# jfjlaros/HUMID

Measured on AMD Instinct MI355X. Metric: reads/sec deduplicated, 10M PE150 UMI=8 d=1, higher is better.
Workload: dtype u64; 1 GPU; 10000000 reads/GPU x 1 GPU (one shuffled read set of 10000000 reads, sliced by input order), PE150 UMI=8 in header -> 24-nt packed words (8+8+8), d=1, directional clustering; synthetic molecules=N/4, family 1+Geom(3), p_sub=1e-3, p_N=1e-4; reads_per_gpu=10000000, word_nt=24, distance=1, method=directional

## Files before the change

humid_amd/csrc/humid_hip.hip:

```cpp
#include "pipeline.hip.h"
#include "kernels_best.hip.h"
#include "kernels_consensus.hip.h"

static std::string g_err;
extern "C" __attribute__((visibility("hidden"))) void humid_set_global_error(const char *text) { g_err = text ? text : ""; }

extern "C" {

uint32_t humid_abi_version(void) { return HUMID_ABI_VERSION; }

int humid_device_count(void) {
  int n = 0;
  if (hipGetDeviceCount(&n) != hipSuccess) return 0;
  return n;
}

const char *humid_last_error(const humid_ctx *ctx) { return ctx ? ctx->err.c_str() : g_err.c_str(); }

int humid_ctx_create(humid_ctx **out, int device, void *stream) {
  humid_ctx *c = nullptr;
  if (!out) return fail(nullptr, HUMID_E_INVALID, "out is null");
  *out = nullptr;
  int ndev = 0;
  hipError_t e = hipGetDeviceCount(&ndev);
// ... 112 lines not shown
    c->kr_force_log2 = (u32)value;
    return HUMID_OK;
  }
  if (strcmp(key, "whitelist_coop") == 0) {
    c->wl_coop = value != 0;
    return HUMID_OK;
  }
  if (strcmp(key, "tile_partition") == 0) {
    c->use_tile_partition = value != 0;
    return HUMID_OK;
  }
  if (strcmp(key, "coop_big") == 0) {
    c->coop_big = value != 0;
    return HUMID_OK;
  }
  if (strcmp(key, "kernel_timing") == 0) {
    c->kev_on = value != 0;
    return HUMID_OK;
  }
  if (strcmp(key, "test_fail_before_gather") == 0) {
    c->x_test_fail_after = (int)value;
    return HUMID_OK;
  }
  if (strcmp(key, "records8") == 0) {
    c->use_rec8 = value != 0;
    return HUMID_OK;
  }
  if (strcmp(key, "compact_graph") == 0) {
    c->use_compact = value != 0;
    return HUMID_OK;
  }
  if (strcmp(key, "group_buckets") == 0) {
    c->group_buckets = value != 0;
    return HUMID_OK;
  }
  if (strcmp(key, "padded_partition") == 0) {
    c->pt_padded = value != 0;
    return HUMID_OK;
  }
  if (strcmp(key, "force_comm") == 0) {
    c->force_comm = value != 0;
    return HUMID_OK;
  }
  if (strcmp(key, "bucket_walk") == 0) {
    if (value < 0 || value > (1 << 24)) return fail(c, HUMID_E_INVALID, "bucket_walk must be 0 (no limit) .. 2^24");
    c->walk_max = (u32)value;
    return HUMID_OK;
  }
  if (strcmp(key, "plan_segments") == 0) {
    if (value < 0 || value > 32) return fail(c, HUMID_E_INVALID, "plan_segments must be 0 (auto) .. 32");
    c->force_segments = (u32)value;
    return HUMID_OK;
  }
  return fail(c, HUMID_E_INVALID, "unknown option '%s'", key);
}

int humid_dedup_run_device(humid_ctx *c, const uint64_t *d_words, const uint8_t *d_filtered,
                           uint64_t n_reads, uint32_t word_nt, uint32_t distance, uint32_t method,
                           uint32_t *d_cluster_id, uint8_t *d_keep, humid_summary *summary) {
  if (!c) return fail(nullptr, HUMID_E_INVALID, "ctx is null");
  return with_word_type(word_nt, [&](auto *w) {
    return run_device(c, (decltype(w))d_words, d_filtered, n_reads, word_nt, distance, method, d_cluster_id, d_keep, summary);
  });
}

int humid_dedup_run_grouped_device(humid_ctx *c, const uint64_t *d_words, const uint32_t *d_group,
// ... 806 lines not shown
```

humid_amd/csrc/kernels_cgraph.hip.h:

```cpp
#ifndef HUMID_KERNELS_CGRAPH_HIP_H
#define HUMID_KERNELS_CGRAPH_HIP_H

#include "common.hip.h"
#include "kernels_graph.hip.h"
#include "kernels_cluster.hip.h"

#define ER_REGIONS 64u
#define ER_STRIDE 32u
struct EdgeRegs {
  u64 *e;
  u32 cap_r;
  u32 *cur;
  const u64 *far;
  u32 n_far;
};
__device__ __forceinline__ u32 er_count(const EdgeRegs &er, u32 r) {
  if (r == ER_REGIONS) return er.n_far;
  const u32 c = er.cur[r * ER_STRIDE];
  return c < er.cap_r ? c : er.cap_r;
}
__device__ __forceinline__ u64 *er_at(const EdgeRegs &er, u32 r, u32 k) {
  return r == ER_REGIONS ? (u64 *)er.far + k : er.e + (size_t)r * er.cap_r + k;
}

// ... 27 lines not shown
    return (u32)(__popc(x.x) + __popc(x.y) + __popc(x.z) + __popc(x.w) + __popc(y.x) + __popc(y.y) + __popc(y.z) + __popc(y.w));
  }
};

static __global__ void __launch_bounds__(256)
k_bits_blocks(const u32 *__restrict__ bits, u32 n_blk, u32 *__restrict__ cnt) {
  HUMID_GUARD_LAST_VGPR();
  const u32 b = blockIdx.x * blockDim.x + threadIdx.x;
  if (b > n_blk) return;
  if (b == n_blk) { cnt[b] = 0; return; }
  const uint4 *p = (const uint4 *)(bits + 8 * (size_t)b);
  const uint4 x = p[0], y = p[1];
  cnt[b] = (u32)(__popc(x.x) + __popc(x.y) + __popc(x.z) + __popc(x.w) + __popc(y.x) + __popc(y.y) + __popc(y.z) + __popc(y.w));
}

#define ZERO_MAX 8
struct ZeroList {
  u32 *p[ZERO_MAX];
  u32 n[ZERO_MAX];
};
static __global__ void __launch_bounds__(256)
k_zero_many(ZeroList z) {
  HUMID_GUARD_LAST_VGPR();
  const u32 stride = gridDim.x * blockDim.x;
#pragma unroll
  for (u32 q = 0; q < ZERO_MAX; q++) {
    u32 *p = z.p[q];
    const u32 n = z.n[q];
    for (u32 i = blockIdx.x * blockDim.x + threadIdx.x; i < n; i += stride) p[i] = 0;
  }
}

#define PA_PPT 4u
template <bool PASS0, class WT>
__global__ void __launch_bounds__(256)
k_pairs_append(const WT *__restrict__ W, const u32 *__restrict__ V, u32 n, WT mask, EarlierMasksT<WT> em, u32 cb,
               u32 distance, u32 walk_max, EdgeRegs er, u32 *bits, ull *big, u32 *overflow,
               const u32 *__restrict__ n_valid = nullptr) {
  HUMID_GUARD_LAST_VGPR();
  __shared__ u32 lds[8];
  __shared__ u32 s_base;
  PH_DECL;
  PH(0);
  if (n_valid && *n_valid < n) n = *n_valid;
  const u32 i0 = blockIdx.x * (PA_PPT * 256u) + threadIdx.x;
  u32 found[PA_PPT], first_off[PA_PPT], jend[PA_PPT];
  WT wi[PA_PPT], w1[PA_PPT];
#pragma unroll
  for (u32 q = 0; q < PA_PPT; q++) {
    const u32 i = i0 + q * 256u;
    found[q] = 0; first_off[q] = 0; jend[q] = 0;
    if (i < n) {
      wi[q] = W[i];
      w1[q] = W[i + 1 < n ? i + 1 : i];
    }
  }
  u32 total_found = 0;
#pragma unroll
  for (u32 q = 0; q < PA_PPT; q++) {
    const u32 i = i0 + q * 256u;
    if (i >= n) continue;
    jend[q] = (walk_max && n - i > walk_max + 1) ? i + walk_max + 1 : n;
    u32 j = i + 1;
    for (; j < jend[q]; j++) {
      const WT x = w_xor(wi[q], j == i + 1 ? w1[q] : W[j]);
      if (w_hits(x, mask)) break;
      if (w_mismatch(x) > distance) continue;
      bool first = true;
#pragma unroll
      for (u32 t = 0; t < MAX_COMBOS; t++)
        first = first && !(t < cb && !w_hits(x, em.m[t]));
      if (!first) continue;
      if (!found[q]) first_off[q] = j - i;
      found[q]++;
    }
    if (big && j == jend[q] && jend[q] < n && !w_hits(w_xor(wi[q], W[jend[q]]), mask)) atomicOr(big, 1ull << cb);
    total_found += found[q];
  }
  PH(1);
  const u32 lane = threadIdx.x & 63, wv = threadIdx.x >> 6;
  u32 incl = total_found;
  incl = wave_incl_scan(incl);
  if (lane == 63) lds[wv] = incl;
  __syncthreads();
  u32 before = 0, total = 0;
#pragma unroll
  for (u32 k = 0; k < 4; k++) { if (k < wv) before += lds[k]; total += lds[k]; }
  PH(2);
  if (total == 0) { PH(3); PH(4); PH_END(5, 4, (blockIdx.x & 15u) == 5u); return; }
  const u32 region = blockIdx.x % ER_REGIONS;
  if (threadIdx.x == 0) s_base = atomicAdd(&er.cur[region * ER_STRIDE], total);
  __syncthreads();
  PH(3);
  if (threadIdx.x == 0) { PH(4); PH_END(5, 4, (blockIdx.x & 15u) == 5u); }
  if (!total_found) return;
  u32 at = s_base + before + incl - total_found;
  if (at + total_found > er.cap_r) { *overflow = 1; if (at >= er.cap_r) return; }
  u64 *out = er.e + (size_t)region * er.cap_r;
#pragma unroll
  for (u32 q = 0; q < PA_PPT; q++) {
    if (!found[q]) continue;
    const u32 i = i0 + q * 256u;
    const u32 ri = PASS0 ? i : V[i];
    auto emit = [&](u32 j) {
      if (at >= er.cap_r) return;
      const u32 rj = PASS0 ? j : V[j];
      out[at++] = ri < rj ? (((u64)ri << 32) | rj) : (((u64)rj << 32) | ri);
      atomicOr(&bits[rj >> 5], 1u << (rj & 31));
    };
    atomicOr(&bits[ri >> 5], 1u << (ri & 31));
    if (found[q] == 1) { emit(i + first_off[q]); continue; }
    for (u32 j = i + first_off[q]; j < jend[q]; j++) {
      const WT x = w_xor(wi[q], W[j]);
      if (w_hits(x, mask)) break;
      if (w_mismatch(x) > distance) continue;
      bool first = true;
#pragma unroll
      for (u32 t = 0; t < MAX_COMBOS; t++)
        first = first && !(t < cb && !w_hits(x, em.m[t]));
      if (first) emit(j);
    }
  }
}

static __global__ void __launch_bounds__(256)
k_mark_pairs(const u64 *__restrict__ pairs, u32 n_pairs, u32 n_leaves, u32 *bits, u32 *bad) {
  HUMID_GUARD_LAST_VGPR();
  const u32 k = blockIdx.x * blockDim.x + threadIdx.x;
  if (k >= n_pairs) return;
  const u64 e = pairs[k];
  const u32 a = (u32)(e >> 32), b = (u32)e;
  if (a >= n_leaves || b >= n_leaves || a == b) { *bad = 1; return; }
  atomicOr(&bits[a >> 5], 1u << (a & 31));
  atomicOr(&bits[b >> 5], 1u << (b & 31));
}

static __global__ void __launch_bounds__(256)
k_nodes_init(BitRank br, u32 n_words, const u32 *__restrict__ s_cnt, u32 *__restrict__ nodes, u32 *__restrict__ ncnt,
             u32 *__restrict__ deg, u32 *__restrict__ parent, u32 *__restrict__ csize, u32 *__restrict__ cur, u32 n_blk) {
  HUMID_GUARD_LAST_VGPR();
  const u32 w = blockIdx.x * blockDim.x + threadIdx.x;
  if (w == 0) deg[br.blk[n_blk]] = 0;
  if (w >= n_words) return;
  u32 x = br.bits[w];
  if (!x) return;
  u32 c = br_rank(br, w << 5);
  while (x) {
    const u32 bit = (u32)__ffs((int)x) - 1u;
    x &= x - 1u;
    const u32 u = (w << 5) | bit;
    nodes[c] = u;
    if (s_cnt) ncnt[c] = s_cnt[u];
    deg[c] = 0; parent[c] = c; csize[c] = 0; cur[c] = 0;
    c++;
  }
}
// ... 236 lines not shown
```

humid_amd/csrc/kernels_part.hip.h:

```cpp
#ifndef HUMID_KERNELS_PART_HIP_H
#define HUMID_KERNELS_PART_HIP_H

#include "common.hip.h"
#include "kernels_count.hip.h"

#define PT_THREADS 1024u
#define PT_TILE 8192u
#define PT_IPT (PT_TILE / PT_THREADS)
#define PT_MAXBINS 512u
#define PT_MAXBINS1 1024u

struct PtInput {
  const u64 *words;
  const u8 *filtered;
  u64 rlo, rhi;
  u32 check_range;
  PartKeyOp key;
};
__device__ __forceinline__ bool pt_load(const PtInput &in, u32 r, u64 &key) {
  if (in.filtered && in.filtered[r]) return false;
  const u64 w = in.words[r];
  if (in.check_range && (w < in.rlo || w > in.rhi)) return false;
  key = in.key(w);
  return true;
// ... 196 lines not shown
    const u32 bin = sbin[s];
    const u32 within = s - loff[bin];
    if (within >= room[bin]) continue;
    const u32 d = goff[bin] + within;
    k_out[d] = skey[s];
    v_out[d] = sval[s];
  }
}

template <class SRC>
__global__ void __launch_bounds__(1024)
k_pt_hist2(SRC src, const u64 *__restrict__ k_in, const u32 *__restrict__ tprefix, const u32 *__restrict__ cbase, u32 d1,
           u32 d2, u32 *__restrict__ hist_fine, u32 cap1) {
  HUMID_GUARD_LAST_VGPR();
  __shared__ u32 h[PT_MAXBINS];
  __shared__ u32 s_c, s_beg, s_cnt;
  if (blockIdx.x >= tprefix[1u << d1]) return;
  const u32 nb = 1u << d2;
  if (threadIdx.x == 0) {
    u32 c, b, n;
    pt_tile_of(tprefix, cbase, 1u << d1, blockIdx.x, cap1, c, b, n);
    s_c = c; s_beg = b; s_cnt = n;
  }
  for (u32 b = threadIdx.x; b < nb; b += PT_THREADS) h[b] = 0;
  __syncthreads();
  const u32 beg = s_beg, n = s_cnt;
  for (u32 j = threadIdx.x; j < n; j += PT_THREADS)
    atomicAdd(&h[(u32)(src.key(k_in[beg + j]) >> (64 - d1 - d2)) & (nb - 1)], 1u);
  __syncthreads();
  for (u32 b = threadIdx.x; b < nb; b += PT_THREADS)
    if (h[b]) atomicAdd(&hist_fine[(s_c << d2) | b], h[b]);
}

#define GF_THREADS 1024u
#define GF_MAXBITS 15u
#define GF_SMALL 7872u
#define GF_MID 32768u
template <class SRC, int SIZE>
__global__ void __launch_bounds__(GF_THREADS, SIZE == 0 ? 8 : 4)
k_group_fine(SRC src, const u64 *__restrict__ k_in, const u32 *__restrict__ v_in, const u32 *__restrict__ cbase, u32 d1,
             u32 d2, u64 *__restrict__ k_out, u32 *__restrict__ v_out, u32 cap1) {
  HUMID_GUARD_LAST_VGPR();
  constexpr bool BIG = SIZE == 2;
  constexpr u32 INV_WORDS = SIZE == 0 ? GF_SMALL / 2u + 16u : (1u << (GF_MAXBITS - 1)) + 16u;
  __shared__ u32 gf_lds[BIG ? (1u << GF_MAXBITS) + 16 : (1u << (GF_MAXBITS - 1)) + INV_WORDS];
  const u32 nb = 1u << d2, c = blockIdx.x;
  PH_DECL;
  PH(0);
  const u32 beg = cbase[c], end = cbase[c + 1];
  if (beg >= end) return;
  const u32 n = end - beg;
  if ((n <= GF_SMALL ? 0 : (n <= GF_MID ? 1 : 2)) != SIZE) return;
  const u32 ibeg = cap1 ? c * cap1 : beg;
  k_in += ibeg; v_in += ibeg; k_out += beg; v_out += beg;
  u32 *wsum = BIG ? gf_lds + (1u << GF_MAXBITS) : gf_lds + (1u << (GF_MAXBITS - 1)) + INV_WORDS - 16;
  const u32 lane = threadIdx.x & 63, wv = threadIdx.x >> 6;
  auto fine = [&](u64 w) { return (u32)(src.key(w) >> (64 - d1 - d2)) & (nb - 1); };
  if (!BIG) {
    unsigned short *inv = (unsigned short *)(gf_lds + (1u << (GF_MAXBITS - 1)));
    constexpr u32 GF_RPT = 8;
    u64 kk[GF_RPT];
    u32 ff[GF_RPT];
    if constexpr (SIZE == 0) {
#pragma unroll
      for (u32 q = 0; q < GF_RPT; q++) {
        const u32 j = threadIdx.x + q * GF_THREADS;
        kk[q] = j < n ? k_in[j] : 0ull;
      }
    }
    for (u32 b = threadIdx.x; b < (1u << (GF_MAXBITS - 1)); b += GF_THREADS) gf_lds[b] = 0;
    __syncthreads();
    PH(1);
    if constexpr (SIZE == 0) {
#pragma unroll
      for (u32 q = 0; q < GF_RPT; q++) {
        const u32 j = threadIdx.x + q * GF_THREADS;
        ff[q] = fine(kk[q]);
        if (j < n) atomicAdd(&gf_lds[ff[q] >> 1], 1u << (16 * (ff[q] & 1)));
// ... 31 lines not shown
    PH(4);
    if constexpr (SIZE == 0) {
      u32 oldq[GF_RPT];
#pragma unroll
      for (u32 q = 0; q < GF_RPT; q++) {
        const u32 j = threadIdx.x + q * GF_THREADS;
        oldq[q] = j < n ? atomicAdd(&gf_lds[ff[q] >> 1], 1u << (16 * (ff[q] & 1))) : 0u;
      }
#pragma unroll
      for (u32 q = 0; q < GF_RPT; q++) {
        const u32 j = threadIdx.x + q * GF_THREADS;
        if (j < n) inv[(oldq[q] >> (16 * (ff[q] & 1))) & 0xffffu] = (unsigned short)j;
      }
      PH(5);
      __syncthreads();
      PH(6);
      u32 jj[GF_RPT], vo[GF_RPT];
      u64 ko[GF_RPT];
#pragma unroll
      for (u32 t = 0; t < GF_RPT; t++) {
        const u32 q = threadIdx.x + t * GF_THREADS;
        jj[t] = q < n ? inv[q] : 0u;
      }
#pragma unroll
      for (u32 t = 0; t < GF_RPT; t++) {
        const u32 q = threadIdx.x + t * GF_THREADS;
        if (q < n) { ko[t] = k_in[jj[t]]; vo[t] = v_in[jj[t]]; }
      }
#pragma unroll
      for (u32 t = 0; t < GF_RPT; t++) {
        const u32 q = threadIdx.x + t * GF_THREADS;
        if (q < n) { k_out[q] = ko[t]; v_out[q] = vo[t]; }
      }
      PH(7);
      PH_END(4, 7, (c & 7u) == 3u);
      return;
    }
    for (u32 j = threadIdx.x; j < n; j += GF_THREADS) {
      const u32 f = fine(k_in[j]);
      const u32 old = atomicAdd(&gf_lds[f >> 1], 1u << (16 * (f & 1)));
      inv[(old >> (16 * (f & 1))) & 0xffffu] = (unsigned short)j;
    }
    __syncthreads();
    for (u32 q = threadIdx.x; q < n; q += GF_THREADS) {
      const u32 j = inv[q];
      k_out[q] = k_in[j];
      v_out[q] = v_in[j];
    }
    return;
  }
  for (u32 b = threadIdx.x; b < nb; b += GF_THREADS) gf_lds[b] = 0;
  __syncthreads();
  for (u32 j = threadIdx.x; j < n; j += GF_THREADS) atomicAdd(&gf_lds[fine(k_in[j])], 1u);
  __syncthreads();
  const u32 per = nb >= GF_THREADS ? nb / GF_THREADS : 1u;
  const u32 b0 = threadIdx.x * per;
  u32 mine = 0;
  if (b0 < nb)
    for (u32 q = 0; q < per; q++) mine += gf_lds[b0 + q];
  u32 incl = mine;
  incl = wave_incl_scan(incl);
  if (lane == 63) wsum[wv] = incl;
  __syncthreads();
  u32 run = incl - mine;
  for (u32 q = 0; q < wv; q++) run += wsum[q];
  if (b0 < nb)
// ... 141 lines not shown
```

humid_amd/csrc/pipeline.hip.h:

```cpp
#ifndef HUMID_PIPELINE_HIP_H
#define HUMID_PIPELINE_HIP_H

#include <fcntl.h>
#include <sys/mman.h>
#include <sys/stat.h>
#include <unistd.h>

#include <atomic>
#include <cerrno>
#include <chrono>
#include <type_traits>
#include <utility>

#include "common.hip.h"
#include "prims.hip.h"
#include "kernels_count.hip.h"
#include "kernels_part.hip.h"
#include "kernels_part8.hip.h"
#include "kernels_graph.hip.h"
#include "kernels_cluster.hip.h"
#include "kernels_cgraph.hip.h"
#include "kernels_map.hip.h"
#include "kernels_xchg.hip.h"
#include "kernels_wide.hip.h"
// ... 78 lines not shown
  DBuf opos, own_packed, owner, owner_sorted, perm, small;
  DBuf pc, poff, share_edges;
  DBuf own_words;
  DBuf heads;
  DBuf small_roots;
  DBuf big_runs;
  DBuf had;
  DBuf e_kx, e_vx, e_ky, e_vy, e_raw, e_sorted, e_edges, e_head, e_hpos;
  DBuf e_runlo, e_nch, e_choff, e_pc2, e_poff2;
  bool edit = false;
  DBuf xr_heads, xr_send, xr_zero;
  DBuf xr_hist, xr_recv, xr_eloc, xr_got, xr_eall, xr_ret;
  DBuf x_slot, x_slot_s, x_cnt, x_cnts, x_rec, x_ncnt, x_route, x_creator, x_base, x_mark, x_markcr, x_scan, x_lcid, x_lismax,
       x_items, x_w, x_id, x_ids, x_ends, x_ends_s, x_head, x_hpos, x_nodes, x_cedges;
  DBuf w_sorted, w_head, w_hpos, w_start, w_heads;
  DBuf cg_edges, cg_cur, cg_far, cg_bits, cg_nbits, cg_blk, cg_nblk, cg_nodes, cg_ncnt, cg_deg, cg_off, cg_idx, cg_parent, cg_csize,
       cg_curs, cg_cl_of, cg_maxleaf, cg_cl_size;
  u64 cg_ecap = 0;
  bool use_compact = true;
  bool cg_valid = false;
  bool cg_expanded = false;
  u32 cg_M = 0, cg_nblocks = 0;
  DBuf xo_gw, xo_gc;
  DBuf xo_regs, xo_inv;
  u64 xr_ecap = 0;
  DBuf xo_send, xo_int, xo_cross, xo_sel, xo_selall, xo_parent, xo_flag, xo_xroot, xo_xcbits, xo_xcblk, xo_xcid, xo_xcall, xo_ldeg, xo_cnt;
  DBuf pw_a, pw_ai, pw_b, pw_bi;
  DBuf p8_a, p8_b, p8_cur, p8_status;
  bool use_rec8 = true;
  bool last_rec8 = false;
  const u32 *rec_cursor2 = nullptr;
  DBuf pt_work, unperm_rec, route_tiles;
  bool group_buckets = true;
  bool pt_padded = true;
  bool use_tile_partition = true;
  bool last_part_tiled = false;
  int x_test_fail_after = -1, x_gathers = 0;
  bool x_hist_done = false, x_peer_failed = false;
  bool route_checked = true;
  const u32 *route_bad = nullptr;
  bool last_unperm_tiled = false;
  bool oc_valid = false, oc_fits = false;
  u32 oc_n = 0, oc_nt = 0;
  u64 oc_lo = 0, oc_scale = 0;
  u32 n_parts = 0;
  bool stage_map_timed = false;
  bool last_count_sorted = false;
  u32 g_wpr = 1;
  bool slots_done = false;
  int count_mode = 0;
  u32 force_segments = 0;
  bool force_comm = false;
  u32 walk_max = PT2_TILE;
  bool coop_big = true;
  bool last_count_lds = false;
  bool last_count_ordered = false;
  int count_order = -1;
  u32 gk_nt = 0;
  u32 gk_epoch = 0;
  u32 gk_word_nt = 0, gk_leaf_nt = 0;
  DBuf gk_words, gk_group_in, gk_bad;
  u32 kr_n = 0;
  u32 kr_cap_log2 = 0;
  u32 kr_force_log2 = 0;
  u32 kr_last_log2 = 0, kr_redo = 0;
  DBuf kr_table, kr_raw, kr_rawslot, kr_keys, kr_slot, kr_key_in;
// ... 890 lines not shown
                         const BigRun **d_runs_out, u32 cap_n = 0) {
  hipStream_t st = c->stream;
  const u32 cap = (cap_n ? cap_n : n) / (walk_max + 2) + 1;
  ENSURE(c->big_runs, (size_t)MAX_COMBOS * cap * sizeof(BigRun) + 16);
  u32 *d_n = (u32 *)((char *)c->big_runs.p + (size_t)MAX_COMBOS * cap * sizeof(BigRun));
  BigRun *d_runs = c->big_runs.as<BigRun>() + (size_t)slot * cap;
  HIPCHK(hipMemsetAsync(d_n, 0, 4, st));
  hipLaunchKernelGGL(k_big_runs<WT>, dim3(blocks_for(n)), dim3(256), 0, st, W, n, mask, walk_max, d_runs, cap, d_n);
  u32 n_runs = 0;
  HIPCHK(hipMemcpyAsync(&n_runs, d_n, 4, hipMemcpyDeviceToHost, st));
  HIPCHK(hipStreamSynchronize(st));
  if (n_runs > cap) return fail(c, HUMID_E_INVALID, "more large buckets (%u) than fit the input (%u)", n_runs, cap);
  runs.resize(n_runs);
  if (n_runs) HIPCHK(hipMemcpy(runs.data(), d_runs, (size_t)n_runs * sizeof(BigRun), hipMemcpyDeviceToHost));
  std::sort(runs.begin(), runs.end(), [](const BigRun &x, const BigRun &y) { return x.start < y.start; });
  ull tiles = 0;
  for (BigRun &x : runs) {
    const ull nt = ((ull)x.len + PT2_TILE - 1) / PT2_TILE;
    x.tile0 = tiles;
    tiles += nt * (nt + 1) / 2;
  }
  runs.push_back(BigRun{0u, 0u, tiles});
  if (n_runs) HIPCHK(hipMemcpy(d_runs, runs.data(), (size_t)n_runs * sizeof(BigRun), hipMemcpyHostToDevice));
  *d_runs_out = d_runs;
  return HUMID_OK;
}

static ComboFields plan_fields(const ComboPlan &plan, u32 cb) {
  ComboFields cf;
  cf.nf = plan.nfield[cb];
  for (u32 f = 0; f < MAX_FIELDS; f++) { cf.shift[f] = plan.shift[cb][f]; cf.width[f] = plan.width[cb][f]; }
  return cf;
}
template <class SRC, class WT>
static int group_words_by_stretch(humid_ctx *c, const ComboPlan &plan, u32 cb, const WT *W, u32 n, u64 *ws, u32 *vs, bool *done,
                                  bool may_pad = false) {
  hipStream_t st = c->stream;
  u32 bit_n = 0;
  for (u32 f = 0; f < plan.nfield[cb]; f++) bit_n += plan.width[cb][f];
  *done = c->group_buckets && plan.nfield[cb] >= 1 && bit_n >= 2 && bit_n <= 24 && n >= 4096;
  c->gf_valid = nullptr;
  if (!*done) return HUMID_OK;
  const u32 d1 = bit_n >= 18 ? 9u : (bit_n + 1) / 2, d2 = bit_n - d1;
  const u32 nb1 = 1u << d1;
  const bool padded = may_pad && c->gf_padded;
  const u32 cap1 = padded ? n / nb1 + n / nb1 / 4 + 1024 : 0u;
  const size_t room = padded ? (size_t)nb1 * cap1 : (size_t)n;
  ENSURE(c->pt_work, (size_t)(1024 + 513 + 513 + 516) * 4);
  u32 *hist1 = c->pt_work.as<u32>(), *cursor1 = hist1 + 512, *cbase = cursor1 + 512, *tprefix = cbase + 513, *dummy = tprefix + 513;
  if (padded) {
    if (!c->gf_cur.p) {
      ENSURE(c->gf_cur, 512 * 4);
      HIPCHK(hipMemsetAsync(c->gf_cur.p, 0, 512 * 4, st));
    }
    cursor1 = c->gf_cur.as<u32>();
  } else HIPCHK(hipMemsetAsync(c->pt_work.p, 0, 1024 * 4, st));
  ENSURE(c->seg_k0, room * 8);
  ENSURE(c->seg_v0, room * 4);
  const SRC src{W, plan_fields(plan, cb), bit_n};
  const u32 tiles1 = (n + PT_TILE - 1) / PT_TILE;
  if (!padded) {
    hipLaunchKernelGGL(k_pt_hist1<SRC>, dim3(tiles1 < 512 ? tiles1 : 512), dim3(1024), 0, st, src, n, d1, hist1);
    hipLaunchKernelGGL(k_pt_scan1, dim3(1), dim3(1024), 0, st, (const u32 *)hist1, d1, 0u, cbase, tprefix, dummy, dummy + 513, 0u);
  }
  static const bool gs_small = getenv("HUMID_GS_THREADS") ? atoi(getenv("HUMID_GS_THREADS")) == 512 : false;
  if (gs_small)
    hipLaunchKernelGGL((k_pt_scatter<1, SRC, 512>), dim3((n + 4095) / 4096), dim3(512), 0, st, src, n, (const u64 *)nullptr,
                       (const u32 *)nullptr, (const u32 *)nullptr, (const u32 *)nullptr, d1, d2, (const u32 *)cbase, cursor1,
                       c->seg_k0.as<u64>(), c->seg_v0.as<u32>(), (u32 *)nullptr, cap1, &c->d_ctr[CTR_GOVER]);
  else
    hipLaunchKernelGGL((k_pt_scatter<1, SRC>), dim3(tiles1), dim3(1024), 0, st, src, n, (const u64 *)nullptr,
                       (const u32 *)nullptr, (const u32 *)nullptr, (const u32 *)nullptr, d1, d2, (const u32 *)cbase, cursor1,
                       c->seg_k0.as<u64>(), c->seg_v0.as<u32>(), (u32 *)nullptr, cap1, &c->d_ctr[CTR_GOVER]);
  if (padded)
    hipLaunchKernelGGL(k_pt_scan1, dim3(1), dim3(1024), 0, st, (const u32 *)cursor1, d1, 0u, cbase, tprefix, dummy, dummy + 513, cap1, cursor1);
  c->gf_valid = padded ? (const u32 *)(cbase + nb1) : (const u32 *)nullptr;
  const u32 largest = padded ? cap1 : n;
  hipLaunchKernelGGL((k_group_fine<SRC, 0>), dim3(nb1), dim3(GF_THREADS), 0, st, src,
                     (const u64 *)c->seg_k0.as<u64>(), (const u32 *)c->seg_v0.as<u32>(), (const u32 *)cbase, d1, d2, ws, vs, cap1);
  if (largest > GF_SMALL)
    hipLaunchKernelGGL((k_group_fine<SRC, 1>), dim3(nb1), dim3(GF_THREADS), 0, st, src,
                       (const u64 *)c->seg_k0.as<u64>(), (const u32 *)c->seg_v0.as<u32>(), (const u32 *)cbase, d1, d2, ws, vs, cap1);
  if (largest > GF_MID)
    hipLaunchKernelGGL((k_group_fine<SRC, 2>), dim3(nb1), dim3(GF_THREADS), 0, st, src,
                       (const u64 *)c->seg_k0.as<u64>(), (const u32 *)c->seg_v0.as<u32>(), (const u32 *)cbase, d1, d2, ws, vs, cap1);
  HIPCHK(hipGetLastError());
  return HUMID_OK;
}

static int sort_words_by_stretch(humid_ctx *c, const ComboPlan &plan, u32 cb, const u64 *W, u32 n, u64 *ws, u32 *vs, bool *done) {
  u32 bit_lo = 0, bit_n = 0;
  bool stretch = plan.nfield[cb] >= 1;
  for (u32 f = 0; stretch && f < plan.nfield[cb]; f++) {
    if (f + 1 < plan.nfield[cb] && plan.shift[cb][f] != plan.shift[cb][f + 1] + plan.width[cb][f + 1]) stretch = false;
    bit_n += plan.width[cb][f];
    bit_lo = plan.shift[cb][f];
  }
  *done = stretch && bit_n >= 1 && bit_lo + bit_n <= 64;
  if (!*done) return HUMID_OK;
  return sort_pairs_in<u64, u32>(c, PtrIn<u64>{W}, ws, IotaIn{}, vs, n, bit_lo, bit_lo + bit_n);
}

template <class WT>
static int bucket_order(humid_ctx *c, const ComboPlan &plan, u32 seg, const WT *g_word, u32 U, WT *ws, u32 *vs, bool may_pad = false) {
  hipStream_t st = c->stream;
  u32 kb = 0;
  for (u32 f = 0; f < plan.nfield[seg]; f++) kb += plan.width[seg][f];
  if (kb == 0) kb = 1;
  bool stretch = false;
  if (std::is_same<WT, u64>::value) {
    TRY((group_words_by_stretch<FieldsSrc, u64>(c, plan, seg, (const u64 *)g_word, U, (u64 *)ws, vs, &stretch, may_pad)));
    if (!stretch) TRY(sort_words_by_stretch(c, plan, seg, (const u64 *)g_word, U, (u64 *)ws, vs, &stretch));
  } else {
    TRY((group_words_by_stretch<FieldsSrcW2, W2>(c, plan, seg, (const W2 *)g_word, U, c->seg_ks.as<u64>(), vs, &stretch, may_pad)));
    if (stretch) hipLaunchKernelGGL(k_gather_bucket_words<WT>, dim3(blocks_for(U)), dim3(256), 0, st, g_word, vs, U, ws, c->gf_valid);
  }
  if (stretch) return HUMID_OK;
  const ComboFields cf = plan_fields(plan, seg);
  if (kb <= 32) {
    hipLaunchKernelGGL((k_combo_keys<u32, WT>), dim3(blocks_for(U)), dim3(256), 0, st, g_word, U, cf,
                       c->seg_k0.as<u32>(), c->seg_v0.as<u32>());
    TRY(sort_pairs<u32, u32>(c, c->seg_k0.as<u32>(), c->seg_ks.as<u32>(), c->seg_v0.as<u32>(), vs, U, 0, kb));
  } else {
    hipLaunchKernelGGL((k_combo_keys<u64, WT>), dim3(blocks_for(U)), dim3(256), 0, st, g_word, U, cf,
                       c->seg_k0.as<u64>(), c->seg_v0.as<u32>());
    TRY(sort_pairs<u64, u32>(c, c->seg_k0.as<u64>(), c->seg_ks.as<u64>(), c->seg_v0.as<u32>(), vs, U, 0, kb));
  }
  hipLaunchKernelGGL(k_gather_bucket_words<WT>, dim3(blocks_for(U)), dim3(256), 0, st, g_word, vs, U, ws);
  HIPCHK(hipGetLastError());
  return HUMID_OK;
}

template <class WT>
struct Walked {
  const WT *W;
  const u32 *V;
  u32 n;
  WT mask;
  u32 cb;
};
template <class WT>
struct PairSearch { EarlierMasksT<WT> em; u32 distance, walk_max; };
struct CsrSink { u32 *deg, *parent; const u32 *nbr_off; u32 *cur, *nbr_idx, *had; const u32 *join_cnt; };
struct EmitSink { u32 *pc; const u32 *poff; u64 *edges; ull *ecount; };
// ... 51 lines not shown
    hipLaunchKernelGGL((k_pairs<decltype(p0)::value, decltype(m)::value, WT>), dim3(blocks_for(n_i)), dim3(256), 0, c->stream, w.W, w.V,
                       w.n, i0, n_i, w.mask, s.em, w.cb, s.distance, (u32 *)nullptr, (u32 *)nullptr, (const u32 *)nullptr,
                       (u32 *)nullptr, (u32 *)nullptr, k.pc, k.poff, k.edges, (u32 *)nullptr, s.walk_max, fill ? nullptr : big,
                       (const u32 *)nullptr);
  });
}
template <class WT>
static void tiles_csr(humid_ctx *c, const PairSearch<WT> &s, const Walked<WT> &w, const BigRun *d_runs, const std::vector<BigRun> &runs,
                      int mode, const CsrSink &k) {
  if (runs.size() < 2) return;
  const ull tiles = runs.back().tile0;
  for_pass_mode<PM_COUNT, PM_FILL>(!w.V, mode == PM_FILL, [&](auto p0, auto m) {
    hipLaunchKernelGGL((k_pairs_tiles<decltype(p0)::value, decltype(m)::value, WT>), dim3((u32)std::min<ull>(tiles, 1u << 20)),
                       dim3(PT2_THREADS), 0, c->stream, w.W, w.V, d_runs, (u32)runs.size() - 1, tiles, s.em, w.cb, s.distance, s.walk_max,
                       k.deg, k.parent, k.nbr_off, k.cur, k.nbr_idx, k.join_cnt, (u64 *)nullptr, (ull *)nullptr, 0u, 0xffffffffu);
  });
}
template <class WT>
static void tiles_emit(humid_ctx *c, const PairSearch<WT> &s, const Walked<WT> &w, const BigRun *d_runs, const std::vector<BigRun> &runs,
                       int mode, const EmitSink &k, u32 i_lo = 0, u32 i_hi = 0xffffffffu) {
  if (runs.size() < 2) return;
  const ull tiles = runs.back().tile0;
  for_pass_mode<PM_EMIT_COUNT, PM_EMIT_FILL>(!w.V, mode == PM_EMIT_FILL, [&](auto p0, auto m) {
    hipLaunchKernelGGL((k_pairs_tiles<decltype(p0)::value, decltype(m)::value, WT>), dim3((u32)std::min<ull>(tiles, 1u << 20)),
                       dim3(PT2_THREADS), 0, c->stream, w.W, w.V, d_runs, (u32)runs.size() - 1, tiles, s.em, w.cb, s.distance, s.walk_max,
                       (u32 *)nullptr, (u32 *)nullptr, (const u32 *)nullptr, (u32 *)nullptr, (u32 *)nullptr, (const u32 *)nullptr,
                       k.edges, k.ecount, i_lo, i_hi);
  });
}
template <class WT>
static void pairs_append(humid_ctx *c, const PairSearch<WT> &s, const Walked<WT> &w, const EdgeRegs &er, u32 *bits, ull *big, u32 *overflow,
                         const u32 *n_valid) {
  const dim3 grid(blocks_for(w.n, PA_PPT * 256)), blk(256);
  if (w.V)
    hipLaunchKernelGGL((k_pairs_append<false, WT>), grid, blk, 0, c->stream, w.W, w.V, w.n, w.mask, s.em, w.cb, s.distance, s.walk_max, er, bits,
                       big, overflow, n_valid);
  else
    hipLaunchKernelGGL((k_pairs_append<true, WT>), grid, blk, 0, c->stream, w.W, w.V, w.n, w.mask, s.em, w.cb, s.distance, s.walk_max, er, bits,
                       big, overflow, n_valid);
}
static void comp_stats(humid_ctx *c, u32 U) {
  hipLaunchKernelGGL(k_comp_stats, dim3(blocks_for(U)), dim3(256), 0, c->stream, c->deg.as<u32>(), c->parent.as<u32>(), U, c->csize.as<u32>());
  hipLaunchKernelGGL(k_comp_count, dim3(512), dim3(256), 0, c->stream, c->deg.as<u32>(), c->parent.as<u32>(), c->csize.as<u32>(), U, c->d_ctr,
                     c->small_roots.as<u32>());
}

template <class WT>
static int stage_graph(humid_ctx *c, const WT *g_word, const u32 *g_cnt, u32 U, u32 word_nt,
                       u32 distance, u32 method, humid_summary &s, u32 &n_pair_segs_out,
                       const u64 *ext_edges = nullptr, u64 n_ext_edges = 0) {
  hipStream_t st = c->stream;
  c->g_word = g_word;
  c->g_wpr = (u32)(sizeof(WT) / 8);
  c->g_cnt = g_cnt;
  c->gU = U;
  c->cg_valid = false;
  ENSURE(c->deg, (size_t)(U + 1) * 4);
  ENSURE(c->nbr_off, (size_t)(U + 1) * 4);
  ENSURE(c->parent, (size_t)U * 4);
  ENSURE(c->csize, (size_t)U * 4);
  ENSURE(c->cur, (size_t)U * 4);
  ENSURE(c->small_roots, ((size_t)U / 3 + 2) * 4);
  HIPCHK(hipMemsetAsync(&c->d_ctr[CTR_EDGES], 0, (CTR_SMALLROOTS - CTR_EDGES + 1) * sizeof(ull), st));
  hipLaunchKernelGGL(k_graph_init, dim3(blocks_for((u64)U + 1)), dim3(256), 0, st, c->parent.as<u32>(),
                     c->deg.as<u32>(), c->csize.as<u32>(), c->cur.as<u32>(), U);
  u64 E = 0, M = 0, Mbig = 0;
  u32 n_pair_segs = 0;
  const ComboPlan plan = make_plan(word_nt - c->gk_nt, distance, U, c->force_segments, true, c->gk_nt);
  const PairSearch<WT> ps = pair_search<WT>(c, plan, distance);
  const bool given = ext_edges != nullptr;
  const bool search = !given && distance > 0 && U > 1;
  const u32 *join_cnt = (method & 1) ? nullptr : g_cnt;
// ... 232 lines not shown
  ENSURE(c->cg_nblk, ((size_t)n_blk + 1) * 4);
  ENSURE(c->cg_cur, (size_t)(ER_REGIONS * ER_STRIDE + 8) * 4);
  ENSURE(c->small_roots, ((size_t)U / 3 + 2) * 4);
  ENSURE(c->small, 64);
  TRY(ensure_seg_scratch<WT>(c, nseg, U));
  u32 *bad = c->cg_cur.as<u32>() + ER_REGIONS * ER_STRIDE;
  const u64 *far = given ? ext_edges : nullptr;
  u64 n_far = given ? n_ext_edges : 0;
  u64 E = 0, M = 0, Mbig = 0;
  CgStatus cgs;
  EdgeRegs er;
  bool ordered_seg[MAX_COMBOS] = {false};
  const u32 *seg_valid[MAX_COMBOS] = {nullptr};
  for (int attempt = 0;; attempt++) {
    if (attempt > 5) return fail(c, HUMID_E_INVALID, "internal: the pair list does not settle");
    if (search && c->cg_ecap == 0) c->cg_ecap = std::max<u64>((u64)U / 4, 4096);
    const u64 ecap = search ? c->cg_ecap : ER_REGIONS;
    if (ecap / ER_REGIONS + 1 > 0xfffffff0ull) return fail(c, HUMID_E_OVERFLOW, "too many neighbour pairs");
    er.cap_r = (u32)((ecap + ER_REGIONS - 1) / ER_REGIONS);
    ENSURE(c->cg_edges, (size_t)ER_REGIONS * er.cap_r * 8);
    er.e = c->cg_edges.as<u64>();
    er.cur = c->cg_cur.as<u32>();
    er.far = far;
    er.n_far = (u32)n_far;
    {
      ZeroList z;
      memset(&z, 0, sizeof z);
      z.p[0] = c->cg_bits.as<u32>(); z.n[0] = n_words;
      z.p[1] = c->cg_nbits.as<u32>(); z.n[1] = n_words;
      z.p[2] = c->cg_cur.as<u32>(); z.n[2] = ER_REGIONS * ER_STRIDE + 8;
      z.p[3] = (u32 *)&c->d_ctr[CTR_EDGES]; z.n[3] = 2 * (CTR_GOVER - CTR_EDGES + 1);
      hipLaunchKernelGGL(k_zero_many, dim3(64), dim3(256), 0, st, z);
    }
    for (u32 seg = 0; seg < nseg; seg++) {
      if (seg) {
        seg_valid[seg] = nullptr;
        if (!ordered_seg[seg]) {
          TRY(bucket_order<WT>(c, plan, seg, g_word, U, seg_ws<WT>(c, seg, U), seg_vs(c, seg, U), true));
          seg_valid[seg] = c->gf_valid;
        }
        ordered_seg[seg] = true;
      }
      if (seg < 8 && c->kev_on) HIPCHK(hipEventRecord(c->kev[20 + 2 * seg], st));
      pairs_append<WT>(c, ps, walked_seg<WT>(c, plan, seg, g_word, U), er, c->cg_bits.as<u32>(), &c->d_ctr[CTR_BIGMASK],
                       (u32 *)&c->d_ctr[CTR_EOVER], seg_valid[seg]);
      if (seg < 8 && c->kev_on) HIPCHK(hipEventRecord(c->kev[21 + 2 * seg], st));
    }
    if (n_far)
      hipLaunchKernelGGL(k_mark_pairs, dim3(blocks_for(n_far)), dim3(256), 0, st, far, (u32)n_far, U, c->cg_bits.as<u32>(), bad);
    CgSource src;
    src.er = er; src.recs = nullptr; src.n_recs = 0; src.cnt_by_id = g_cnt; src.n_ids = U;
    src.pairs_bound = ecap + n_far;
    TRY(cg_build(c, src, method, cgs));
    er = src.er;
    if (cgs.group_over) {
      c->gf_padded = false;
      for (u32 q = 0; q < MAX_COMBOS; q++) ordered_seg[q] = false;
      far = given ? ext_edges : nullptr;
      n_far = given ? n_ext_edges : 0;
      continue;
    }
    if (cgs.overflow) {
      c->cg_ecap = cgs.wanted + cgs.wanted / 2 + ER_REGIONS * 64;
      continue;
    }
    if (given) {
      u32 h_bad = 0;
      HIPCHK(hipMemcpyAsync(&h_bad, bad, 4, hipMemcpyDeviceToHost, st));
      HIPCHK(hipStreamSynchronize(st));
      if (h_bad) return fail(c, HUMID_E_INVALID, "malformed edge list (node index out of range)");
    }
    if (search && cgs.big_mask && !far) {
      const u64 big_mask = cgs.big_mask;
      u64 got = 0;
      for (int phase = 0; phase < 2; phase++) {
        u64 at = 0;
        for (u32 seg = 0; seg < nseg; seg++) {
          if (!(big_mask >> seg & 1)) continue;
          const Walked<WT> w = walked_seg<WT>(c, plan, seg, g_word, U);
          std::vector<BigRun> runs;
          const BigRun *d_runs = nullptr;
          TRY(find_big_runs<WT>(c, w.W, U, w.mask, ps.walk_max, seg, runs, &d_runs));
          if (!runs.back().tile0) continue;
          const ull start = phase ? at : 0;
          HIPCHK(hipMemcpyAsync(&c->d_ctr[CTR_SPECIAL], &start, sizeof(ull), hipMemcpyHostToDevice, st));
          HIPCHK(hipStreamSynchronize(st));
          tiles_emit<WT>(c, ps, w, d_runs, runs, phase ? PM_EMIT_FILL : PM_EMIT_COUNT,
                         EmitSink{nullptr, nullptr, c->cg_far.as<u64>(), &c->d_ctr[CTR_SPECIAL]});
          HIPCHK(hipGetLastError());
          TRY(read_counters(c));
          if (phase == 0) got += c->h_ctr[CTR_SPECIAL]; else at = c->h_ctr[CTR_SPECIAL];
        }
        if (phase == 0) {
          if (got > 0x7fffffffull) return fail(c, HUMID_E_OVERFLOW, "%llu neighbour pairs exceed the 32-bit adjacency offsets", (ull)got);
          ENSURE(c->cg_far, (size_t)(got + 1) * 8);
        }
// ... 611 lines not shown
```

Measured before the change: 15.79 billion reads/s.

## Fuse neighbour-pair search into the small-bin group_fine kernel via LDS words

Refactors the pair-append walk and emit into reusable device helpers, then runs the pair search inside the k_group_fine launch for small padded bins. The grouped words are staged in LDS and walked there, which removes a separate k_pairs_append launch and its global re-read of the segment words. This is on by default for u64 words and can be turned off with a new fused_search option. The fused kernel may take more registers and LDS, which can lower occupancy. It also resets the far edges when a capacity overflow forces a retry.

```diff
diff --git a/humid_amd/csrc/humid_hip.hip b/humid_amd/csrc/humid_hip.hip
--- a/humid_amd/csrc/humid_hip.hip
+++ b/humid_amd/csrc/humid_hip.hip
@@ -168,6 +168,10 @@
   }
   if (strcmp(key, "group_buckets") == 0) {
     c->group_buckets = value != 0;
+    return HUMID_OK;
+  }
+  if (strcmp(key, "fused_search") == 0) {
+    c->fused_search = value != 0;
     return HUMID_OK;
   }
   if (strcmp(key, "padded_partition") == 0) {
diff --git a/humid_amd/csrc/kernels_cgraph.hip.h b/humid_amd/csrc/kernels_cgraph.hip.h
--- a/humid_amd/csrc/kernels_cgraph.hip.h
+++ b/humid_amd/csrc/kernels_cgraph.hip.h
@@ -83,96 +83,152 @@
 }
 
 #define PA_PPT 4u
-template <bool PASS0, class WT>
-__global__ void __launch_bounds__(256)
-k_pairs_append(const WT *__restrict__ W, const u32 *__restrict__ V, u32 n, WT mask, EarlierMasksT<WT> em, u32 cb,
-               u32 distance, u32 walk_max, EdgeRegs er, u32 *bits, ull *big, u32 *overflow,
-               const u32 *__restrict__ n_valid = nullptr) {
-  HUMID_GUARD_LAST_VGPR();
-  __shared__ u32 lds[8];
-  __shared__ u32 s_base;
-  PH_DECL;
-  PH(0);
-  if (n_valid && *n_valid < n) n = *n_valid;
-  const u32 i0 = blockIdx.x * (PA_PPT * 256u) + threadIdx.x;
-  u32 found[PA_PPT], first_off[PA_PPT], jend[PA_PPT];
-  WT wi[PA_PPT], w1[PA_PPT];
-#pragma unroll
-  for (u32 q = 0; q < PA_PPT; q++) {
-    const u32 i = i0 + q * 256u;
-    found[q] = 0; first_off[q] = 0; jend[q] = 0;
-    if (i < n) {
-      wi[q] = W[i];
-      w1[q] = W[i + 1 < n ? i + 1 : i];
-    }
-  }
+
+template <class WT>
+struct WordsGlobal {
+  const WT *W;
+  __device__ __forceinline__ WT operator()(u32 j) const { return W[j]; }
+};
+struct IdxSelf { __device__ __forceinline__ u32 operator()(u32 j) const { return j; } };
+struct IdxGlobal {
+  const u32 *V;
+  __device__ __forceinline__ u32 operator()(u32 j) const { return V[j]; }
+};
+template <class WT>
+struct PairRule {
+  WT mask;
+  EarlierMasksT<WT> em;
+  u32 cb, distance, walk_max;
+};
+template <class WT>
+__device__ __forceinline__ bool pa_pair(WT x, const PairRule<WT> &r) {
+  if (w_mismatch(x) > r.distance) return false;
+  for (u32 t = 0; t < r.cb; t++)
+    if (!w_hits(x, r.em.m[t])) return false;
+  return true;
+}
+__device__ __forceinline__ u32 pa_jend(u32 i, u32 n, u32 walk_max) { return (walk_max && n - i > walk_max + 1) ? i + walk_max + 1 : n; }
+template <class WT, class ACC>
+__device__ __forceinline__ void pa_walk(const ACC &word, WT wi, WT w1, u32 i, u32 n, const PairRule<WT> &r, ull *big, u32 &found, u32 &first_off) {
+  const u32 jend = pa_jend(i, n, r.walk_max);
+  u32 j = i + 1;
+  for (; j < jend; j++) {
+    const WT x = w_xor(wi, j == i + 1 ? w1 : word(j));
+    if (w_hits(x, r.mask)) break;
+    if (!pa_pair(x, r)) continue;
+    if (!found) first_off = j - i;
+    found++;
+  }
+  if (big && j == jend && jend < n && !w_hits(w_xor(wi, word(jend)), r.mask)) atomicOr(big, 1ull << r.cb);
+}
+template <u32 NP, u32 NW, class WT, class ACC, class IDX>
+__device__ __forceinline__ void pa_emit(const ACC &word, const IDX &idx, u32 i0, u32 stride, u32 n, const u32 (&found)[NP],
+                                        const u32 (&first_off)[NP], const PairRule<WT> &r, const EdgeRegs &er, u32 *bits, u32 *overflow,
+                                        u32 *lds) {
   u32 total_found = 0;
 #pragma unroll
-  for (u32 q = 0; q < PA_PPT; q++) {
-    const u32 i = i0 + q * 256u;
-    if (i >= n) continue;
-    jend[q] = (walk_max && n - i > walk_max + 1) ? i + walk_max + 1 : n;
-    u32 j = i + 1;
-    for (; j < jend[q]; j++) {
-      const WT x = w_xor(wi[q], j == i + 1 ? w1[q] : W[j]);
-      if (w_hits(x, mask)) break;
-      if (w_mismatch(x) > distance) continue;
-      bool first = true;
-#pragma unroll
-      for (u32 t = 0; t < MAX_COMBOS; t++)
-        first = first && !(t < cb && !w_hits(x, em.m[t]));
-      if (!first) continue;
-      if (!found[q]) first_off[q] = j - i;
-      found[q]++;
-    }
-    if (big && j == jend[q] && jend[q] < n && !w_hits(w_xor(wi[q], W[jend[q]]), mask)) atomicOr(big, 1ull << cb);
-    total_found += found[q];
-  }
-  PH(1);
+  for (u32 q = 0; q < NP; q++) total_found += found[q];
   const u32 lane = threadIdx.x & 63, wv = threadIdx.x >> 6;
-  u32 incl = total_found;
-  incl = wave_incl_scan(incl);
+  const u32 incl = wave_incl_scan(total_found);
   if (lane == 63) lds[wv] = incl;
   __syncthreads();
   u32 before = 0, total = 0;
 #pragma unroll
-  for (u32 k = 0; k < 4; k++) { if (k < wv) before += lds[k]; total += lds[k]; }
-  PH(2);
-  if (total == 0) { PH(3); PH(4); PH_END(5, 4, (blockIdx.x & 15u) == 5u); return; }
+  for (u32 k = 0; k < NW; k++) { const u32 x = lds[k]; if (k < wv) before += x; total += x; }
+  if (total == 0) return;
   const u32 region = blockIdx.x % ER_REGIONS;
-  if (threadIdx.x == 0) s_base = atomicAdd(&er.cur[region * ER_STRIDE], total);
+  if (threadIdx.x == 0) lds[NW] = atomicAdd(&er.cur[region * ER_STRIDE], total);
   __syncthreads();
-  PH(3);
-  if (threadIdx.x == 0) { PH(4); PH_END(5, 4, (blockIdx.x & 15u) == 5u); }
   if (!total_found) return;
-  u32 at = s_base + before + incl - total_found;
+  u32 at = lds[NW] + before + incl - total_found;
   if (at + total_found > er.cap_r) { *overflow = 1; if (at >= er.cap_r) return; }
   u64 *out = er.e + (size_t)region * er.cap_r;
 #pragma unroll
-  for (u32 q = 0; q < PA_PPT; q++) {
+  for (u32 q = 0; q < NP; q++) {
     if (!found[q]) continue;
-    const u32 i = i0 + q * 256u;
-    const u32 ri = PASS0 ? i : V[i];
+    const u32 i = i0 + q * stride;
+    const u32 ri = idx(i);
     auto emit = [&](u32 j) {
       if (at >= er.cap_r) return;
-      const u32 rj = PASS0 ? j : V[j];
+      const u32 rj = idx(j);
       out[at++] = ri < rj ? (((u64)ri << 32) | rj) : (((u64)rj << 32) | ri);
       atomicOr(&bits[rj >> 5], 1u << (rj & 31));
     };
     atomicOr(&bits[ri >> 5], 1u << (ri & 31));
     if (found[q] == 1) { emit(i + first_off[q]); continue; }
-    for (u32 j = i + first_off[q]; j < jend[q]; j++) {
-      const WT x = w_xor(wi[q], W[j]);
-      if (w_hits(x, mask)) break;
-      if (w_mismatch(x) > distance) continue;
-      bool first = true;
-#pragma unroll
-      for (u32 t = 0; t < MAX_COMBOS; t++)
-        first = first && !(t < cb && !w_hits(x, em.m[t]));
-      if (first) emit(j);
-    }
-  }
-}
+    const WT wi = word(i);
+    const u32 jend = pa_jend(i, n, r.walk_max);
+    for (u32 j = i + first_off[q]; j < jend; j++) {
+      const WT x = w_xor(wi, word(j));
+      if (w_hits(x, r.mask)) break;
+      if (pa_pair(x, r)) emit(j);
+    }
+  }
+}
+
+template <bool PASS0, class WT>
+__global__ void __launch_bounds__(256)
+k_pairs_append(const WT *__restrict__ W, const u32 *__restrict__ V, u32 n, PairRule<WT> rule, EdgeRegs er, u32 *bits, ull *big, u32 *overflow,
+               const u32 *__restrict__ n_valid = nullptr) {
+  HUMID_GUARD_LAST_VGPR();
+  __shared__ u32 lds[5];
+  PH_DECL;
+  PH(0);
+  if (n_valid && *n_valid < n) n = *n_valid;
+  const u32 i0 = blockIdx.x * (PA_PPT * 256u) + threadIdx.x;
+  const WordsGlobal<WT> word{W};
+  u32 found[PA_PPT], first_off[PA_PPT];
+  WT wi[PA_PPT], w1[PA_PPT];
+#pragma unroll
+  for (u32 q = 0; q < PA_PPT; q++) {
+    const u32 i = i0 + q * 256u;
+    found[q] = 0; first_off[q] = 0;
+    if (i < n) {
+      wi[q] = W[i];
+      w1[q] = W[i + 1 < n ? i + 1 : i];
+    }
+  }
+#pragma unroll
+  for (u32 q = 0; q < PA_PPT; q++) {
+    const u32 i = i0 + q * 256u;
+    if (i < n) pa_walk(word, wi[q], w1[q], i, n, rule, big, found[q], first_off[q]);
+  }
+  PH(1);
+  if (PASS0) pa_emit<PA_PPT, 4>(word, IdxSelf{}, i0, 256u, n, found, first_off, rule, er, bits, overflow, lds);
+  else pa_emit<PA_PPT, 4>(word, IdxGlobal{V}, i0, 256u, n, found, first_off, rule, er, bits, overflow, lds);
+  PH(2); PH(3); PH(4);
+  PH_END(5, 4, (blockIdx.x & 15u) == 5u);
+}
+
+struct WordsLds {
+  const u64 *sw;
+  __device__ __forceinline__ u64 operator()(u32 j) const { return sw[j]; }
+};
+struct IdxGrouped {
+  const unsigned short *inv;
+  const u32 *v_in;
+  __device__ __forceinline__ u32 operator()(u32 j) const { return v_in[inv[j]]; }
+};
+struct PairSearchDev {
+  static constexpr bool on = true;
+  PairRule<u64> rule;
+  EdgeRegs er;
+  u32 *bits;
+  ull *big;
+  u32 *overflow;
+  template <u32 NP, u32 T>
+  __device__ __forceinline__ void in_bin(const u64 *sw, u32 n, const unsigned short *inv, const u32 *v_in, u32 *scratch) const {
+    const WordsLds word{sw};
+    u32 found[NP], first_off[NP];
+#pragma unroll
+    for (u32 q = 0; q < NP; q++) {
+      const u32 i = threadIdx.x + q * T;
+      found[q] = 0; first_off[q] = 0;
+      if (i < n) pa_walk(word, sw[i], sw[i + 1 < n ? i + 1 : i], i, n, rule, big, found[q], first_off[q]);
+    }
+    pa_emit<NP, T / 64u>(word, IdxGrouped{inv, v_in}, threadIdx.x, T, n, found, first_off, rule, er, bits, overflow, scratch);
+  }
+};
 
 static __global__ void __launch_bounds__(256)
 k_mark_pairs(const u64 *__restrict__ pairs, u32 n_pairs, u32 n_leaves, u32 *bits, u32 *bad) {
diff --git a/humid_amd/csrc/kernels_part.hip.h b/humid_amd/csrc/kernels_part.hip.h
--- a/humid_amd/csrc/kernels_part.hip.h
+++ b/humid_amd/csrc/kernels_part.hip.h
@@ -252,18 +252,21 @@
     if (h[b]) atomicAdd(&hist_fine[(s_c << d2) | b], h[b]);
 }
 
+struct NoSearch { static constexpr bool on = false; };
 #define GF_THREADS 1024u
 #define GF_MAXBITS 15u
 #define GF_SMALL 7872u
 #define GF_MID 32768u
-template <class SRC, int SIZE>
+template <class SRC, int SIZE, class SEARCH = NoSearch>
 __global__ void __launch_bounds__(GF_THREADS, SIZE == 0 ? 8 : 4)
 k_group_fine(SRC src, const u64 *__restrict__ k_in, const u32 *__restrict__ v_in, const u32 *__restrict__ cbase, u32 d1,
-             u32 d2, u64 *__restrict__ k_out, u32 *__restrict__ v_out, u32 cap1) {
-  HUMID_GUARD_LAST_VGPR();
+             u32 d2, u64 *__restrict__ k_out, u32 *__restrict__ v_out, u32 cap1, SEARCH srch = SEARCH()) {
+  HUMID_GUARD_LAST_VGPR();
+  static_assert(SIZE == 0 || !SEARCH::on, "the search rides in the launch of the small bins");
+  static_assert(GF_SMALL * 2u + 32u <= (1u << (GF_MAXBITS - 1)), "the grouped words and the emit's words fit the counter area");
   constexpr bool BIG = SIZE == 2;
   constexpr u32 INV_WORDS = SIZE == 0 ? GF_SMALL / 2u + 16u : (1u << (GF_MAXBITS - 1)) + 16u;
-  __shared__ u32 gf_lds[BIG ? (1u << GF_MAXBITS) + 16 : (1u << (GF_MAXBITS - 1)) + INV_WORDS];
+  __shared__ __attribute__((aligned(8))) u32 gf_lds[BIG ? (1u << GF_MAXBITS) + 16 : (1u << (GF_MAXBITS - 1)) + INV_WORDS];
   const u32 nb = 1u << d2, c = blockIdx.x;
   PH_DECL;
   PH(0);
@@ -361,6 +364,16 @@
         const u32 q = threadIdx.x + t * GF_THREADS;
         if (q < n) { k_out[q] = ko[t]; v_out[q] = vo[t]; }
       }
+      if constexpr (SEARCH::on) {
+        u64 *sw = (u64 *)gf_lds;
+#pragma unroll
+        for (u32 t = 0; t < GF_RPT; t++) {
+          const u32 q = threadIdx.x + t * GF_THREADS;
+          if (q < n) sw[q] = ko[t];
+        }
+        __syncthreads();
+        srch.template in_bin<GF_RPT, GF_THREADS>(sw, n, inv, v_in, gf_lds + 2u * GF_SMALL);
+      }
       PH(7);
       PH_END(4, 7, (c & 7u) == 3u);
       return;
diff --git a/humid_amd/csrc/pipeline.hip.h b/humid_amd/csrc/pipeline.hip.h
--- a/humid_amd/csrc/pipeline.hip.h
+++ b/humid_amd/csrc/pipeline.hip.h
@@ -134,6 +134,7 @@
   const u32 *rec_cursor2 = nullptr;
   DBuf pt_work, unperm_rec, route_tiles;
   bool group_buckets = true;
+  bool fused_search = true;
   bool pt_padded = true;
   bool use_tile_partition = true;
   bool last_part_tiled = false;
@@ -1090,9 +1091,16 @@
   for (u32 f = 0; f < MAX_FIELDS; f++) { cf.shift[f] = plan.shift[cb][f]; cf.width[f] = plan.width[cb][f]; }
   return cf;
 }
+struct GroupRide {
+  PairSearchDev group;
+  bool did_group = false;
+  hipEvent_t ev_group[2] = {nullptr, nullptr};
+};
+static void group_fine_with_search(humid_ctx *c, const FieldsSrc &src, const u64 *k0, const u32 *v0, const u32 *cbase, u32 d1, u32 d2, u64 *ws,
+                                   u32 *vs, u32 cap1, const PairSearchDev &s);
 template <class SRC, class WT>
 static int group_words_by_stretch(humid_ctx *c, const ComboPlan &plan, u32 cb, const WT *W, u32 n, u64 *ws, u32 *vs, bool *done,
-                                  bool may_pad = false) {
+                                  bool may_pad = false, GroupRide *ride = nullptr) {
   hipStream_t st = c->stream;
   u32 bit_n = 0;
   for (u32 f = 0; f < plan.nfield[cb]; f++) bit_n += plan.width[cb][f];
@@ -1122,6 +1130,7 @@
     hipLaunchKernelGGL(k_pt_scan1, dim3(1), dim3(1024), 0, st, (const u32 *)hist1, d1, 0u, cbase, tprefix, dummy, dummy + 513, 0u);
   }
   static const bool gs_small = getenv("HUMID_GS_THREADS") ? atoi(getenv("HUMID_GS_THREADS")) == 512 : false;
+  const bool ride_ok = ride && std::is_same<SRC, FieldsSrc>::value && padded && cap1 <= GF_SMALL;
   if (gs_small)
     hipLaunchKernelGGL((k_pt_scatter<1, SRC, 512>), dim3((n + 4095) / 4096), dim3(512), 0, st, src, n, (const u64 *)nullptr,
                        (const u32 *)nullptr, (const u32 *)nullptr, (const u32 *)nullptr, d1, d2, (const u32 *)cbase, cursor1,
@@ -1134,6 +1143,14 @@
     hipLaunchKernelGGL(k_pt_scan1, dim3(1), dim3(1024), 0, st, (const u32 *)cursor1, d1, 0u, cbase, tprefix, dummy, dummy + 513, cap1, cursor1);
   c->gf_valid = padded ? (const u32 *)(cbase + nb1) : (const u32 *)nullptr;
   const u32 largest = padded ? cap1 : n;
+  if (ride_ok) {
+    if constexpr (std::is_same<SRC, FieldsSrc>::value) {
+      if (ride->ev_group[0]) HIPCHK(hipEventRecord(ride->ev_group[0], st));
+      group_fine_with_search(c, src, c->seg_k0.as<u64>(), c->seg_v0.as<u32>(), cbase, d1, d2, ws, vs, cap1, ride->group);
+      if (ride->ev_group[1]) HIPCHK(hipEventRecord(ride->ev_group[1], st));
+      ride->did_group = true;
+    }
+  } else
   hipLaunchKernelGGL((k_group_fine<SRC, 0>), dim3(nb1), dim3(GF_THREADS), 0, st, src,
                      (const u64 *)c->seg_k0.as<u64>(), (const u32 *)c->seg_v0.as<u32>(), (const u32 *)cbase, d1, d2, ws, vs, cap1);
   if (largest > GF_SMALL)
@@ -1160,14 +1177,15 @@
 }
 
 template <class WT>
-static int bucket_order(humid_ctx *c, const ComboPlan &plan, u32 seg, const WT *g_word, u32 U, WT *ws, u32 *vs, bool may_pad = false) {
+static int bucket_order(humid_ctx *c, const ComboPlan &plan, u32 seg, const WT *g_word, u32 U, WT *ws, u32 *vs, bool may_pad = false,
+                        GroupRide *ride = nullptr) {
   hipStream_t st = c->stream;
   u32 kb = 0;
   for (u32 f = 0; f < plan.nfield[seg]; f++) kb += plan.width[seg][f];
   if (kb == 0) kb = 1;
   bool stretch = false;
   if (std::is_same<WT, u64>::value) {
-    TRY((group_words_by_stretch<FieldsSrc, u64>(c, plan, seg, (const u64 *)g_word, U, (u64 *)ws, vs, &stretch, may_pad)));
+    TRY((group_words_by_stretch<FieldsSrc, u64>(c, plan, seg, (const u64 *)g_word, U, (u64 *)ws, vs, &stretch, may_pad, ride)));
     if (!stretch) TRY(sort_words_by_stretch(c, plan, seg, (const u64 *)g_word, U, (u64 *)ws, vs, &stretch));
   } else {
     TRY((group_words_by_stretch<FieldsSrcW2, W2>(c, plan, seg, (const W2 *)g_word, U, c->seg_ks.as<u64>(), vs, &stretch, may_pad)));
@@ -1285,12 +1303,19 @@
 static void pairs_append(humid_ctx *c, const PairSearch<WT> &s, const Walked<WT> &w, const EdgeRegs &er, u32 *bits, ull *big, u32 *overflow,
                          const u32 *n_valid) {
   const dim3 grid(blocks_for(w.n, PA_PPT * 256)), blk(256);
+  const PairRule<WT> rule{w.mask, s.em, w.cb, s.distance, s.walk_max};
   if (w.V)
-    hipLaunchKernelGGL((k_pairs_append<false, WT>), grid, blk, 0, c->stream, w.W, w.V, w.n, w.mask, s.em, w.cb, s.distance, s.walk_max, er, bits,
-                       big, overflow, n_valid);
+    hipLaunchKernelGGL((k_pairs_append<false, WT>), grid, blk, 0, c->stream, w.W, w.V, w.n, rule, er, bits, big, overflow, n_valid);
   else
-    hipLaunchKernelGGL((k_pairs_append<true, WT>), grid, blk, 0, c->stream, w.W, w.V, w.n, w.mask, s.em, w.cb, s.distance, s.walk_max, er, bits,
-                       big, overflow, n_valid);
+    hipLaunchKernelGGL((k_pairs_append<true, WT>), grid, blk, 0, c->stream, w.W, w.V, w.n, rule, er, bits, big, overflow, n_valid);
+}
+static PairSearchDev pairs_append_dev(const PairSearch<u64> &s, u64 mask, u32 cb, const EdgeRegs &er, u32 *bits, ull *big, u32 *overflow) {
+  return PairSearchDev{PairRule<u64>{mask, s.em, cb, s.distance, s.walk_max}, er, bits, big, overflow};
+}
+static void group_fine_with_search(humid_ctx *c, const FieldsSrc &src, const u64 *k0, const u32 *v0, const u32 *cbase, u32 d1, u32 d2, u64 *ws,
+                                   u32 *vs, u32 cap1, const PairSearchDev &s) {
+  hipLaunchKernelGGL((k_group_fine<FieldsSrc, 0, PairSearchDev>), dim3(1u << d1), dim3(GF_THREADS), 0, c->stream, src, k0, v0, cbase, d1, d2, ws,
+                     vs, cap1, s);
 }
 static void comp_stats(humid_ctx *c, u32 U) {
   hipLaunchKernelGGL(k_comp_stats, dim3(blocks_for(U)), dim3(256), 0, c->stream, c->deg.as<u32>(), c->parent.as<u32>(), U, c->csize.as<u32>());
@@ -1589,19 +1614,33 @@
       z.p[3] = (u32 *)&c->d_ctr[CTR_EDGES]; z.n[3] = 2 * (CTR_GOVER - CTR_EDGES + 1);
       hipLaunchKernelGGL(k_zero_many, dim3(64), dim3(256), 0, st, z);
     }
-    for (u32 seg = 0; seg < nseg; seg++) {
-      if (seg) {
-        seg_valid[seg] = nullptr;
-        if (!ordered_seg[seg]) {
-          TRY(bucket_order<WT>(c, plan, seg, g_word, U, seg_ws<WT>(c, seg, U), seg_vs(c, seg, U), true));
-          seg_valid[seg] = c->gf_valid;
-        }
-        ordered_seg[seg] = true;
-      }
+    auto search_alone = [&](u32 seg) -> int {
       if (seg < 8 && c->kev_on) HIPCHK(hipEventRecord(c->kev[20 + 2 * seg], st));
       pairs_append<WT>(c, ps, walked_seg<WT>(c, plan, seg, g_word, U), er, c->cg_bits.as<u32>(), &c->d_ctr[CTR_BIGMASK],
                        (u32 *)&c->d_ctr[CTR_EOVER], seg_valid[seg]);
       if (seg < 8 && c->kev_on) HIPCHK(hipEventRecord(c->kev[21 + 2 * seg], st));
+      return HUMID_OK;
+    };
+    const bool ride_on = c->fused_search && std::is_same<WT, u64>::value;
+    for (u32 seg = 0; seg < nseg; seg++) {
+      bool searched = false;
+      if (seg) {
+        seg_valid[seg] = nullptr;
+        if (!ordered_seg[seg]) {
+          GroupRide ride;
+          if constexpr (std::is_same<WT, u64>::value) {
+            if (ride_on) {
+              ride.group = pairs_append_dev(ps, w_from<u64>(plan.mask[seg]), seg, er, c->cg_bits.as<u32>(), &c->d_ctr[CTR_BIGMASK], (u32 *)&c->d_ctr[CTR_EOVER]);
+              if (seg < 8 && c->kev_on) { ride.ev_group[0] = c->kev[20 + 2 * seg]; ride.ev_group[1] = c->kev[21 + 2 * seg]; }
+            }
+          }
+          TRY(bucket_order<WT>(c, plan, seg, g_word, U, seg_ws<WT>(c, seg, U), seg_vs(c, seg, U), true, ride_on ? &ride : nullptr));
+          seg_valid[seg] = c->gf_valid;
+          searched = ride.did_group;
+        }
+        ordered_seg[seg] = true;
+      }
+      if (!searched) TRY(search_alone(seg));
     }
     if (n_far)
       hipLaunchKernelGGL(k_mark_pairs, dim3(blocks_for(n_far)), dim3(256), 0, st, far, (u32)n_far, U, c->cg_bits.as<u32>(), bad);
@@ -1619,6 +1658,7 @@
     }
     if (cgs.overflow) {
       c->cg_ecap = cgs.wanted + cgs.wanted / 2 + ER_REGIONS * 64;
+      if (!given) { far = nullptr; n_far = 0; }
       continue;
     }
     if (given) {
```

Result: faster. 16.73 billion reads/s (median of 6 runs) (+5.9%).
